# facebookresearch/CPC_audio

Hardware: AMD Instinct MI355X
Metric: audio-seconds/sec (train step) (higher is better)
Workload: dtype f32 (conv GEMMs and the GRU forward recurrence: fp32 operands as 2 scaled fp16 pieces -- the inputs of conv1/conv2 stored that way --, 3 fp16 MFMAs per product; GRU backward recurrence and the criterion's dz gather-GEMM: f32 MFMAs; InfoNCE scores: 2 fp16 pieces; other GEMMs: 3 bf16 pieces, 6 bf16 MF

## Files before the change

cpc_audio_amd/_lib.py:

```python
import ctypes
import os
import threading

_HERE = os.path.dirname(os.path.abspath(__file__))
LIB_PATH = os.path.join(_HERE, "lib", "libcpc_hip.so")
DEFAULT_GRU_MODE = 2
DEFAULT_GRU_XCD_LOCAL = 1
DEFAULT_GRU_POLL_PLAIN = 15
DEFAULT_MFMA_MODE = 3
EXPECTED_ABI = 16
DEFAULT_DMA_PIPELINE = 2
DEFAULT_WGRAD_DMA_STAGES = 4
DEFAULT_CONV_SMALL_PIPE = 1
DEFAULT_GRU_WGRAD_STREAM = 1
DEFAULT_NCE_FUSED = 2
DEFAULT_INDEX_PREP_GROUPS = -1
DEFAULT_FWD_NSPLIT = 0
DEFAULT_DGRAD_NSPLIT = 256
DEFAULT_STEP_SCHEDULE = (1, 0)

_P = ctypes.c_void_p
_I = ctypes.c_int
_L = ctypes.c_long
_F = ctypes.c_float

SIGNATURES = {
    "cpc_abi_version": (_I, []),
    "cpc_release_stream": (_I, [_P]),
    "cpc_streams_overlap": (_I, [_P, _P, _P]),
    "cpc_set_mfma_mode": (_I, [_I]),
    "cpc_get_mfma_mode": (_I, []),
    "cpc_device_error_flags": (_I, [_I]),
    "cpc_conv0_forward": (_I, [_P] * 8 + [_I, _I, _P]),
    "cpc_conv0_forward_h2": (_I, [_P] * 9 + [_I, _I, _P]),
    "cpc_h2_encode": (_I, [_P, _P, _L, _P, _P]),
    "cpc_h2_decode": (_I, [_P, _P, _L, _P, _P]),
    "cpc_conv_weight_relayout_h2": (_I, [_P, _P, _I, _P]),
    "cpc_conv_gemm_forward_h2": (_I, [_P] * 11 + [_I] * 6 + [_P]),
    "cpc_set_dma_tile": (_I, [_I]),
    "cpc_set_conv0_tuning": (_I, [_I, _I]),
    "cpc_set_h2_layers": (_I, [_I]),
    "cpc_set_h2_dx": (_I, [_I]),
    "cpc_set_wgrad1_early": (_I, [_I]),
    "cpc_set_dma_layer2": (_I, [_I]),
    "cpc_set_conv_small_tile": (_I, [_I]),
    "cpc_set_dgrad_nsplit": (_I, [_I]),
    "cpc_set_conv_small_pipe": (_I, [_I]),
    "cpc_set_wgrad_dma_groups": (_I, [_I]),
    "cpc_set_wgrad_dma_stages": (_I, [_I]),
    "cpc_set_wgrad_dma_min_rows": (_I, [_I]),
    "cpc_set_gemm_split": (_I, [_I]),
    "cpc_set_gemm_dma": (_I, [_I]),
# ... 82 lines not shown
    "cpc_pred_conv_backward": (_I, [_P] * 8 + [_I] * 5 + [_F, _I, _P]),
    "cpc_probe_layout": (_I, [_I, _I, _P]),
    "cpc_probe_train_step": (_I, [_P, _L, _P, _I, _I] + [_P] * 6 + [ctypes.c_double] * 6 + [_P] * 7),
    "cpc_probe_eval": (_I, [_P, _L, _P, _I, _I] + [_P] * 7),
    "cpc_posterior_forward": (_I, [_P, _L, _P, _P, _I, _I, _I, _P, _P, _P]),
    "cpc_abx_layout": (_I, [_I, _I, _I, _L, _P]),
    "cpc_abx_group_scores": (_I, [_P, _P, _P, _I, _L, _I, _I, _I, _P, _P, _P, _I, _P, _I, _I, _P, _P, _P]),
    "cpc_abx_pair_dtw": (_I, [_P, _P, _P, _I, _L, _I, _I, _I, _P, _I, _P, _P]),
    "cpc_abx_dtw": (_I, [_P, _P, _P, _I, _I, _I, _I, _I, _I, _P, _P]),
    "cpc_ctc_decode_layout": (_I, [_I, _I, _I, _I, _P]),
    "cpc_ctc_beam_search": (_I, [_P, _I, _L, _L, _L, _P, _I, _I, _I, _I, _I, _I, _P, _L, _P, _P, _P, _P, _P]),
    "cpc_nw_align_score": (_I, [_P, _L, _P, _I, _P, _L, _P, _I, _I, ctypes.c_double, ctypes.c_double, ctypes.c_double, _I, _P,
                                _P]),
    "cpc_nce_layout": (_I, [_I, _I, _I, _I, _P]),
    "cpc_nce_prepare": (_I, [_P] * 6 + [_I, _I, _I, _I, _P]),
    "cpc_nce_forward": (_I, [_P] * 8 + [_I, _I, _I, _I, _P]),
    "cpc_nce_forward_prepared": (_I, [_P] * 8 + [_I, _I, _I, _I, _P]),
    "cpc_nce_bounds": (_I, [_P, ctypes.c_float, _P, _P, _I, _I, _I, _I, _P]),
    "cpc_nce_forward_streams": (_I, [_P] * 8 + [_I, _I, _I, _I, _I, _P, _P]),
    "cpc_nce_backward_prepare": (_I, [_P] * 5 + [_I, _I, _I, _I, _P]),
    "cpc_nce_backward_prepared": (_I, [_P] * 10 + [_I, _I, _I, _I, _P]),
    "cpc_nce_backward": (_I, [_P] * 12 + [_I, _I, _I, _I, _P]),
    "cpc_nce_backward_streams": (_I, [_P] * 12 + [_I, _I, _I, _I, _P, _P]),
    "cpc_nce_backward_dz": (_I, [_P] * 7 + [_I, _I, _I, _I, _P]),
    "cpc_nce_backward_dwall": (_I, [_P] * 4 + [_I, _I, _I, _I, _P]),
    "cpc_set_nce_fused": (_I, [_I]),
    "cpc_get_nce_fused": (_I, []),
    "cpc_set_nce_grid": (_I, [_I]),
    "cpc_set_nce_debug": (_I, [_I]),
    "cpc_set_nce_rows_apart": (_I, [_I]),
    "cpc_set_nce_heads_dma": (_I, [_I]),
    "cpc_nce_prepare_z": (_I, [_P, _P, _I, _I, _I, _I, _P]),
    "cpc_set_index_prep_groups": (_I, [_I]),
    "cpc_set_gru_wgrad_stream": (_I, [_I]),
    "cpc_nce_padded_negatives": (_I, [_I]),
    "cpc_nce_head_group": (_I, [_I, _I]),
    "cpc_set_step_schedule": (_I, [_I, _I]),
    "cpc_train_step_layout": (_I, [_I, _I, _I, _I, _P]),
    "cpc_train_step_prefetch": (_I, [_P, _P, _P, _I, _I, _I, _I, _P]),
    "cpc_train_step": (_I, [_P, _P, _P, _P, _F] + [_P] * 7 + [_I] * 5 + [_P] * 4),
    "cpc_train_step_tail": (_I, [_P, _P, _I, _I, _I, _I, _I, _P, _P, _P]),
    "cpc_train_step_wait": (_I, [_P, _I, _P]),
    "cpc_set_fwd_nsplit": (_I, [_I, _I]),
    "cpc_set_step_timing": (_I, [_I]),
    "cpc_set_tail_schedule": (_I, [_I]),
    "cpc_get_step_timing": (_I, [_P]),
    "cpc_adam_step": (_I, [_P] * 5 + [_I] + [ctypes.c_double] * 6 + [_P]),
    "cpc_adam_step_capturable": (_I, [_P] * 5 + [_I] + [ctypes.c_double] * 4 + [_P, _P, _P]),
}


class CpcHipError(RuntimeError):
    pass


class Bound:

    def __init__(self, cdll, path):
        self.path = path
        self._cdll = cdll
        missing = []
        for name, (res, args) in SIGNATURES.items():
            try:
                fn = getattr(cdll, name)
            except AttributeError:
                missing.append(name)
# ... 56 lines not shown
```

cpc_audio_amd/csrc/cpc_internal.h:

```cpp
#pragma once
#include "cpc_common.h"
#include "gemm_tile.h"

namespace cpc {

constexpr int kRowsSumGroups = 128;
int rows_sum(const float* part, int nrows, int n, float* tmp, float* out, hipStream_t stream, int G = 1, long part_gs = 0,
             long tmp_gs = 0, long out_gs = 0);
constexpr int kRowsSumMaxJobs = 8;
struct RowsSumJob { const float* part; int nrows; int n; float* tmp; float* out; };
int rows_sum_multi(const RowsSumJob* jobs, int njobs, hipStream_t stream);

struct GemmBounds {
    const float* a = nullptr;
    const float* b = nullptr;
    int a_slots = 1, b_slots = 1;
    long a_gs = 0, b_gs = 0;
};
int absmax_slots(const float* const* x, const long* n, int njobs, float* out, hipStream_t st, const float* cval = nullptr);
int absmax_group(const float* const* x, const long* n, const long* x_gs, int njobs, int G, float* out, long out_gs, hipStream_t st);

struct GemmGroup {
    int G = 1;
    long a = 0, b = 0, bias = 0, c = 0;
// ... 92 lines not shown
                        int* splits_out, hipStream_t st);
int conv_wgrad_dma(const void* dx_h2, const void* x_h2, float* part, const float* dx_bound, const float* x_bound,
                   const float* zeros, int B, int Lin, int k, int s, int p, int* splits_out, hipStream_t st);
int bf16_decode(const void* src, float* dst, long n, hipStream_t st);
int conv0_forward_bf16(const float* wave, const float* w, const float* bias, const float* nw, const float* nb, void* y,
                       float* mean, float* rstd, int B, int L, hipStream_t st);
int conv0_backward(const float* wave, const float* w, const float* bias, const float* nw, const float* nb,
                   const float* mean, const float* rstd, const void* dy, int dy_bf16, float* scratch, float* dW0, float* dB0,
                   float* dNW0, float* dNB0, int B, int L, hipStream_t stream);

int head_row_lse(const float* logits, float* lse, int R, int C, hipStream_t st);
int head_colsum(const float* dl, float* dbp, int R, int C, int kchunk, int Z, hipStream_t st);
constexpr int kCtcNone = 0, kCtcMean = 1, kCtcSum = 2;
int ctc_loss_saved_floats(int B, int T, int C, int Lmax, long* floats);
int ctc_loss_forward(const float* logits, const long long* in_len, const long long* targets, long tgt_stride,
                     const long long* tgt_len, float* saved, float* loss, int B, int T, int C, int Lmax, int blank, int reduction,
                     hipStream_t st);
int ctc_loss_backward(const float* logits, const float* saved, const float* dloss, float* dlogits, int B, int T, int C, int Lmax,
                      int blank, int reduction, hipStream_t st);

template <class T>
int device_flag_fetch(T& sym, int clear, unsigned* out) {
    unsigned v = 0;
    if (hipMemcpyFromSymbol(&v, sym, sizeof(v)) != hipSuccess) return CPC_ERR_ARG;
    if (clear && v) {
        const unsigned zero = 0;
        if (hipMemcpyToSymbol(sym, &zero, sizeof(zero)) != hipSuccess) return CPC_ERR_ARG;
    }
    *out = v;
    return 0;
}
int gru_error_flag_fetch(int clear, unsigned* out);
int nce_error_flag_fetch(int clear, unsigned* out);
int enc_error_flag_fetch(int clear, unsigned* out);
int lstm_error_flag_fetch(int clear, unsigned* out);
int sup_error_flag_fetch(int clear, unsigned* out);
int probe_error_flag_fetch(int clear, unsigned* out);
int abx_error_flag_fetch(int clear, unsigned* out);
int decode_error_flag_fetch(int clear, unsigned* out);
int ctc_error_flag_fetch(int clear, unsigned* out);
int seqnorm_error_flag_fetch(int clear, unsigned* out);
int rnn_error_flag_fetch(int clear, unsigned* out);

static inline long align64l(long v) { return (v + 63) & ~63L; }

}
```

cpc_audio_amd/csrc/nce.hip:

```cpp
#include <algorithm>
#include "cpc_common.h"
#include "cpc_internal.h"
#include "gemm_tile.h"

namespace cpc {

__device__ __forceinline__ float4 ld4(const float* p) { return *reinterpret_cast<const float4*>(p); }
__device__ __forceinline__ float dot4(const float4& a, const float4& b) {
    return fmaf(a.x, b.x, fmaf(a.y, b.y, fmaf(a.z, b.z, a.w * b.w)));
}

struct Gather16 {
    float4 v[4][4];
    __device__ __forceinline__ void issue(const float* const (&rowp)[4]) {
#pragma unroll
        for (int q = 0; q < 4; ++q)
#pragma unroll
            for (int g = 0; g < 4; ++g) v[q][g] = ld4(rowp[q] + 64 * g);
    }
    __device__ __forceinline__ void block(int g, float4* tile, float4 (&out)[4]) const {
        const int lane = threadIdx.x & 63, c = lane & 15, r4 = lane >> 4;
        __builtin_amdgcn_wave_barrier();
#pragma unroll
        for (int q = 0; q < 4; ++q) tile[(4 * q + r4) * 16 + (c ^ (4 * q + r4))] = v[q][g];
// ... 1110 lines not shown
__global__ __launch_bounds__(1024) void nce_scan_kernel(const int* __restrict__ count, int* __restrict__ row_ptr,
                                                        int* __restrict__ cursor, int n) {
    __shared__ int part[1024];
    const int tid = threadIdx.x;
    const int per = (n + 1023) / 1024;
    const int lo = tid * per, hi = min(n, lo + per);
    int s = 0;
    for (int i = lo; i < hi; ++i) s += count[i];
    part[tid] = s;
    __syncthreads();
    for (int off = 1; off < 1024; off <<= 1) {
        const int v = tid >= off ? part[tid - off] : 0;
        __syncthreads();
        part[tid] += v;
        __syncthreads();
    }
    int run = part[tid] - s;
    for (int i = lo; i < hi; ++i) {
        row_ptr[i] = run;
        cursor[i] = run;
        run += count[i];
    }
    if (tid == 1023) row_ptr[n] = part[1023];
}

__global__ __launch_bounds__(256) void nce_fill_kernel(const int* __restrict__ dest, int* __restrict__ cursor,
                                                       int* __restrict__ perm, long total) {
    for (long slot = (long)blockIdx.x * 256 + threadIdx.x; slot < total; slot += (long)gridDim.x * 256) {
        const int pos = atomicAdd(&cursor[dest[slot]], 1);
        perm[pos] = (int)slot;
    }
}

int g_index_prep_groups = -1;
int g_nce_fused = 2;
int g_nce_heads_dma = 1;
int g_nce_dbg = 0;
int g_nce_rows_apart = 1;
int g_nce_grid = -1;

struct NceLayout {
    int W, BW;
    int koff;
    int N, Nv;
    long pred, logits, lse, bounds, tpred, ps, zh, chf, wqh, saved_total;
    long rowstat, tmp, sums, fwd_total;
    long dpred, wallT, part, gscale, V, dS, G, wcat, part_dz, ch, bwd_total;
};

constexpr int kDzSplits = 4;

static thread_local int g_head_off = 0, g_head_total = 0;
static thread_local bool g_zh_ready = false;
static thread_local bool g_wqh_ready = false;

static bool nce_layout(int B, int S, int K, int N, NceLayout& n) {
    const int Ktot = g_head_total > 0 ? g_head_total : K;
    if (B <= 0 || K <= 0 || K > 16 || g_head_off + K > Ktot || S <= Ktot || N <= 0) return false;
    n.Nv = N;
    N = (N + 15) & ~15;
    n.N = N;
    n.koff = g_head_total > 0 ? g_head_off : 0;
    n.W = S - Ktot;
    n.BW = B * n.W;
    long o = 0;
    n.pred = o; o += align64l((long)n.BW * K * kC);
// ... 145 lines not shown
    if (h2) { gb.a = bnd + 128; gb.a_slots = kAmaxSlots; gb.b = bnd + 18; }
    SplitK sk;
    sk.part = scratch + n.part_dz;
    sk.floats = (long)kDzSplits * B * S * kC;
    return nt_gemm(plain_rows(G, B * S, K * kC), wcat, K * kC, nullptr, dz, kC, kC, K * kC, st, 0, 0, gb, GemmGroup(), sk);
}

__global__ __launch_bounds__(256) void nce_scale_tpred_kernel(const float* __restrict__ T, const float* __restrict__ gscale,
                                                              float* __restrict__ dpred, long n4, int K) {
    const long i = (long)blockIdx.x * 256 + threadIdx.x;
    if (i >= n4) return;
    const float g = gscale[(int)((i / (kC / 4)) % K)];
    float4 v = reinterpret_cast<const float4*>(T)[i];
    v.x *= g; v.y *= g; v.z *= g; v.w *= g;
    reinterpret_cast<float4*>(dpred)[i] = v;
}

static int nce_scores_backward(const NceLayout& n, const float* z, const int* ext, const float* saved, const float* gloss,
                               float* scratch, float* dpred, int B, int S, int K, int N, hipStream_t st,
                               const float* fwd_bounds = nullptr, float* dc_tail = nullptr, float* dS = nullptr,
                               bool gscale_done = false) {
    const float* logits = saved + n.logits, *lse = saved + n.lse;
    float* gscale = scratch + n.gscale;
    const float gs = 1.0f / ((float)n.BW * (float)kC);
    if (!gscale_done)
    hipLaunchKernelGGL(nce_gscale_kernel, dim3(dc_tail ? 1 + 128 : 1), dim3(64), 0, st, gloss, gscale, K, gs, fwd_bounds, dc_tail, B,
                       S, n.W);
    hipLaunchKernelGGL(nce_bwd_dpred_kernel, dim3(cdiv(n.BW, 4)), dim3(256), 0, st, z, ext, logits, lse, gscale, dpred, n.BW,
                       n.W, S, K, N, fwd_bounds ? gscale + 64 : (float*)nullptr, dS, n.koff);
    CPC_LAUNCH_CHECK();
    return 0;
}

int nce_error_flag_fetch(int clear, unsigned* out) { return device_flag_fetch(HIP_SYMBOL(g_nce_bad_index), clear, out); }

}

using namespace cpc;

extern "C" int cpc_nce_layout(int B, int S, int K, int N, long* sizes) {
    NceLayout n;
    CPC_RETURN_IF(!nce_layout(B, S, K, N, n), CPC_ERR_SHAPE);
    N = n.N;
    sizes[0] = n.saved_total; sizes[1] = n.fwd_total; sizes[2] = n.bwd_total;
    sizes[3] = n.pred; sizes[4] = n.logits; sizes[5] = n.lse;
    return 0;
}

extern "C" int cpc_nce_padded_negatives(int N) { return N <= 0 ? 0 : (N + 15) & ~15; }

extern "C" int cpc_nce_prepare(const long* batchIdx, const long* seqIdx, int* ext, int* perm, int* row_ptr,
                               int* work, int B, int S, int K, int N, void* stream) {
    NceLayout n;
    CPC_RETURN_IF(!nce_layout(B, S, K, N, n), CPC_ERR_SHAPE);
    N = n.N;
    CPC_RETURN_IF(!batchIdx || !seqIdx || !ext || !perm || !row_ptr || !work, CPC_ERR_ARG);
    hipStream_t st = (hipStream_t)stream;
    const long total = (long)n.BW * (N + K);
    const int rows = B * S;
    int* dest = work;
    int* count = work + total;
    int* cursor = count + rows + 1;
    (void)hipMemsetAsync(count, 0, sizeof(int) * (rows + 1), st);
    long cap = g_index_prep_groups;
    if (cap < 0) {
        int dev = 0, cus = 0;
        if (hipGetDevice(&dev) != hipSuccess || hipDeviceGetAttribute(&cus, hipDeviceAttributeMultiprocessorCount, dev) != hipSuccess) cus = 0;
        cap = cus;
    }
    const auto capped = [cap](long wgs) { return (unsigned)(cap > 0 ? std::min<long>(wgs, cap) : wgs); };
    hipLaunchKernelGGL(nce_rows_kernel, dim3(capped(cdiv(n.BW, 4))), dim3(256), 0, st, batchIdx, seqIdx, ext, B, S, n.W, n.Nv, N);
    hipLaunchKernelGGL(nce_index_kernel, dim3(capped(cdiv(total, 256))), dim3(256), 0, st, ext, dest, count, B, S, n.W, K, N, n.koff);
    hipLaunchKernelGGL(nce_scan_kernel, dim3(1), dim3(1024), 0, st, count, row_ptr, cursor, rows);
    hipLaunchKernelGGL(nce_fill_kernel, dim3(capped(cdiv(total, 256))), dim3(256), 0, st, dest, cursor, perm, total);
    CPC_LAUNCH_CHECK();
    return 0;
}

static int nce_forward(const float* c, const float* z, const float* wall, const int* ext, float* saved, float* scratch,
                       float* losses, float* acc, int B, int S, int K, int N, hipStream_t st, bool bounds_ready,
                       hipStream_t fin = nullptr) {
    NceLayout n;
    CPC_RETURN_IF(!nce_layout(B, S, K, N, n), CPC_ERR_SHAPE);
    N = n.N;
    CPC_RETURN_IF(!c || !z || !wall || !ext || !saved || !scratch || !losses || !acc, CPC_ERR_ARG);
    float* pred = saved + n.pred;
    if (!bounds_ready) {
        const float* xs[3] = {c, wall, nullptr};
        const long ns[3] = {(long)B * S * kC, (long)K * kC * kC, 0};
        int rc = absmax_slots(xs, ns, 3, saved + n.bounds, st);
        if (rc) return rc;
    }
    GemmBounds gb;
    gb.a = saved + n.bounds; gb.a_slots = kAmaxSlots;
    gb.b = saved + n.bounds + kAmaxSlots; gb.b_slots = kAmaxSlots;
    int rc = 0;
    if (nce_heads_dma(K)) {
        if (!(bounds_ready && g_wqh_ready))
            rc = gemm_weight_h2(wall, kC, 1, K * kC, kC, saved + n.wqh, saved + n.bounds + kAmaxSlots, nullptr, 1, 0, 0, 0, 0, st);
        g_wqh_ready = false;
        if (rc) return rc;
        rc = nce_rows_to_h2(c, saved + n.chf, saved + n.bounds, (long)B * S, st);
// ... 191 lines not shown
}

extern "C" int cpc_nce_backward_dwall(const float* c, const float* saved, float* scratch, float* dwall, int B, int S, int K,
                                      int N, void* stream) {
    NceLayout n;
    CPC_RETURN_IF(!nce_layout(B, S, K, N, n), CPC_ERR_SHAPE);
    N = n.N;
    CPC_RETURN_IF(!c || !saved || !scratch || !dwall, CPC_ERR_ARG);
    const bool fused = nce_fused(N) != 0;
    GemmBounds gdw;
    GemmGroup grp;
    if (g_mfma_mode >= 2) {
        gdw.a = fused ? saved + n.bounds + 2 * kAmaxSlots : scratch + n.gscale + 64; gdw.a_slots = kAmaxSlots;
        gdw.b = scratch + n.gscale + 17;
    }
    if (fused) { grp.out_scale = scratch + n.gscale; grp.out_scale_rows = kC; }
    return tn_gemm(plain_rows(fused ? saved + n.tpred : scratch + n.dpred, n.BW, K * kC), K * kC, window_rows(c, B, S, n.W), kC,
                   scratch + n.part, dwall, 0, (hipStream_t)stream, gdw, grp);
}

extern "C" int cpc_nce_head_group(int k0, int k_total) {
    CPC_RETURN_IF(k0 < 0 || k_total < 0 || (k_total == 0 && k0 != 0) || (k_total > 0 && k0 >= k_total), CPC_ERR_ARG);
    g_head_off = k0;
    g_head_total = k_total;
    return 0;
}

extern "C" int cpc_set_index_prep_groups(int n) {
    CPC_RETURN_IF(n < -1, CPC_ERR_ARG);
    g_index_prep_groups = n;
    return 0;
}

extern "C" int cpc_set_nce_fused(int on) {
    CPC_RETURN_IF(on < 0 || on > 3, CPC_ERR_ARG);
    g_nce_fused = on;
    return 0;
}
extern "C" int cpc_get_nce_fused(void) { return g_nce_fused; }
extern "C" int cpc_set_nce_heads_dma(int on) { g_nce_heads_dma = on ? 1 : 0; return 0; }
extern "C" int cpc_set_nce_rows_apart(int on) { g_nce_rows_apart = on ? 1 : 0; return 0; }
extern "C" int cpc_set_nce_debug(int mask) { g_nce_dbg = mask; return 0; }

extern "C" int cpc_set_nce_grid(int wgs) {
    CPC_RETURN_IF(wgs < -1, CPC_ERR_ARG);
    g_nce_grid = wgs;
    return 0;
}

extern "C" int cpc_nce_prepare_z(const float* z, float* saved, int B, int S, int K, int N, void* stream) {
    NceLayout n;
    CPC_RETURN_IF(!nce_layout(B, S, K, N, n), CPC_ERR_SHAPE);
    CPC_RETURN_IF(!z || !saved, CPC_ERR_ARG);
    if (nce_fused(n.N) < 2) return 0;
    g_zh_ready = true;
    return nce_prepare_zh(n, z, saved, B, S, (hipStream_t)stream);
}
```

cpc_audio_amd/csrc/train_step.hip:

```cpp
#include "cpc_common.h"
#include "cpc_internal.h"

namespace cpc {
namespace {

constexpr int kEncParams = 20, kGruParams = 8;

struct StepLayout {
    int S, W;
    long enc[22], gru[3], nce[6], coef;
    long enc_saved, enc_fscr, z, gru_saved, gru_fscr, c, gcoef, nce_saved, nce_fscr, ext, perm, row_ptr, work;
    long nce_bscr, dc, dz, gru_bscr, dx, enc_bscr, total;
};

bool step_layout(int B, int L, int K, int N, StepLayout& s) {
    if (B <= 0 || cpc_encoder_layout(B, L, s.enc) != 0) return false;
    s.S = (int)s.enc[7];
    s.W = s.S - K;
    if (s.W <= 0 || cpc_gru_layout(B, s.S, 2, s.gru) != 0 || cpc_nce_layout(B, s.S, K, N, s.nce) != 0) return false;
    s.coef = cpc_gru_coef_floats(B, s.S, 2);
    if (s.coef <= 0) return false;
    const int Np = cpc_nce_padded_negatives(N);
    const long act = (long)B * s.S * kC, slots = (long)B * s.W * (Np + K), rows = (long)B * s.S;
    long o = 0;
    auto take = [&](long n) { const long at = o; o += align64l(n); return at; };
    s.enc_saved = take(s.enc[0]); s.enc_fscr = take(std::max(1L, s.enc[1])); s.z = take(act);
    s.gru_saved = take(s.gru[0]); s.gru_fscr = take(s.gru[1]); s.c = take(act); s.gcoef = take(s.coef);
    s.nce_saved = take(s.nce[0]); s.nce_fscr = take(s.nce[1]);
    s.ext = take((long)B * s.W * Np); s.perm = take(slots); s.row_ptr = take(rows + 1); s.work = take(slots + 2 * rows + 2);
    s.nce_bscr = take(s.nce[2]); s.dc = take(act); s.dz = take(act);
    s.gru_bscr = take(s.gru[2]); s.dx = take(act); s.enc_bscr = take(s.enc[2]);
    s.total = o;
    return true;
}

__global__ __launch_bounds__(256) void add_inplace_kernel(float* __restrict__ a, const float* __restrict__ b, long n4) {
    const long i = (long)blockIdx.x * 256 + threadIdx.x;
    if (i >= n4) return;
    float4 x = reinterpret_cast<float4*>(a)[i];
    const float4 y = reinterpret_cast<const float4*>(b)[i];
    x.x += y.x; x.y += y.y; x.z += y.z; x.w += y.w;
    reinterpret_cast<float4*>(a)[i] = x;
}

int g_prep_point = 1;
int g_no_early = 0;
int g_weight_prep_apart = 0;
int g_gru_wgrad_prep = 1;
int g_dz_early = 0;

inline bool rec(hipEvent_t e, hipStream_t s) { return hipEventRecord(e, s) == hipSuccess; }
inline bool wait(hipStream_t s, hipEvent_t e) { return hipStreamWaitEvent(s, e, 0) == hipSuccess; }

int g_step_timing = 0;
hipEvent_t g_timers[10];
bool g_timers_made = false;

struct HookScope {
    StepHooks saved;
    HookScope() : saved(step_hooks()) {}
    ~HookScope() { step_hooks() = saved; }
};

}

void enc_set_after_conv0_event(hipEvent_t ev);
void enc_set_forward_event(int layer, hipEvent_t ev);
void enc_set_weight_prep_stream(hipStream_t st, hipEvent_t done);

}

using namespace cpc;

extern "C" int cpc_set_gru_wgrad_stream(int on_prep) {
    g_gru_wgrad_prep = on_prep ? 1 : 0;
    return 0;
}

extern "C" int cpc_set_step_schedule(int prep_point, int dz_early) {
    CPC_RETURN_IF(prep_point < 0 || prep_point > 3 || dz_early < 0 || dz_early > 7, CPC_ERR_ARG);
    g_prep_point = prep_point;
    g_dz_early = dz_early & 1;
    g_no_early = (dz_early >> 1) & 1;
    g_weight_prep_apart = (dz_early >> 2) & 1;
    return 0;
}

extern "C" int cpc_train_step_layout(int B, int L, int K, int N, long* sizes) {
    StepLayout s;
    CPC_RETURN_IF(!sizes || !step_layout(B, L, K, N, s), CPC_ERR_SHAPE);
    sizes[0] = s.total; sizes[1] = s.z; sizes[2] = s.c; sizes[3] = s.S;
    sizes[4] = s.ext; sizes[5] = s.dz; sizes[6] = s.dc; sizes[7] = s.dx;
    return 0;
}

extern "C" int cpc_train_step(const float* wave, const long* batchIdx, const long* seqIdx, const float* h0, float c_bound,
                              const float* const* params, float* const* grads, const float* gloss, float* workspace,
                              float* losses, float* acc, float* hN, int B, int L, int K, int N, int phases, void* main_stream,
                              void* side_stream, void* prep_stream, void* wgrad_stream) {
    StepLayout s;
    CPC_RETURN_IF(!step_layout(B, L, K, N, s), CPC_ERR_SHAPE);
    CPC_RETURN_IF(!wave || !params || !grads || !workspace || (phases & ~31) || !(phases & 3), CPC_ERR_ARG);
    CPC_RETURN_IF(((phases & 4) && !(phases & 2)) || ((phases & 8) && !(phases & 1)), CPC_ERR_ARG);
    hipStream_t M = (hipStream_t)main_stream, S0 = (hipStream_t)side_stream, S1 = (hipStream_t)prep_stream,
                S2 = (hipStream_t)wgrad_stream;
    hipEvent_t* pool = stream_events(M);
    CPC_RETURN_IF(!pool, CPC_ERR_ARG);
    HookScope scope;
    StepHooks& hk = step_hooks();
    hk.parity = (phases & 16) ? 1 : 0;
    hk.weights_ready = (phases & 8) != 0;
    hk.conv1_wait[0] = (phases & 8) ? pool[kEvNextConv1] : nullptr;
    hk.conv1_wait[1] = (phases & 8) ? pool[kEvNextRest] : nullptr;
    hk.open_tail = (phases & 4) != 0 && S2 != M;
    hk.sums_stream = hk.open_tail && S1 != M ? S1 : nullptr;
    hk.timers = (g_step_timing && g_timers_made) ? g_timers : nullptr;
    hipEvent_t* ev = pool + 12;
    float* ws = workspace;
    const float* const* enc_p = params;
    const float* const* gru_p = params + kEncParams;
    const float* wall = params[kEncParams + kGruParams];
    float* const* enc_g = grads;
    float* const* gru_g = grads + kEncParams;
    float* dwall = grads[kEncParams + kGruParams];
    float* z = ws + s.z, *c = ws + s.c, *coef = ws + s.gcoef, *dz = ws + s.dz, *dc = ws + s.dc, *dx = ws + s.dx;
    int* ext = reinterpret_cast<int*>(ws + s.ext), *perm = reinterpret_cast<int*>(ws + s.perm);
    int* row_ptr = reinterpret_cast<int*>(ws + s.row_ptr), *work = reinterpret_cast<int*>(ws + s.work);
    const int S = s.S;
    int rc = 0;
    if (phases & 1) {
        CPC_RETURN_IF((batchIdx == nullptr) != (seqIdx == nullptr) || !gloss || !losses || !acc || !hN, CPC_ERR_ARG);
        CPC_RETURN_IF(!rec(ev[0], M) || !wait(S1, ev[0]), CPC_ERR_ARG);
        if (phases & 8) CPC_RETURN_IF(!wait(S0, pool[kEvNextRest]), CPC_ERR_ARG);
        const bool bounds_early = c_bound > 0.f;
        const bool early = bounds_early && !g_no_early;
        auto prepare = [&]() -> int {
            int r = batchIdx ? cpc_nce_prepare(batchIdx, seqIdx, ext, perm, row_ptr, work, B, S, K, N, S0) : 0;
            if (r) return r;
            if (bounds_early) r = cpc_nce_bounds(nullptr, c_bound, wall, ws + s.nce_saved, B, S, K, N, S0);
            if (r) return r;
            if (early) r = cpc_nce_backward_prepare(wall, ws + s.nce_saved, gloss, ws + s.nce_bscr, dc, B, S, K, N, S0);
            if (r) return r;
            return rec(ev[1], S0) ? 0 : CPC_ERR_ARG;
        };
        if (g_prep_point == 0) {
            CPC_RETURN_IF(!wait(S0, ev[0]), CPC_ERR_ARG);
            if ((rc = prepare())) return rc;
        }
        if (g_prep_point == 3) enc_set_forward_event(1, ev[6]);
        else enc_set_after_conv0_event(g_prep_point == 1 ? ev[6] : nullptr);
        enc_set_weight_prep_stream(g_weight_prep_apart ? S1 : nullptr, ev[8]);
        rc = cpc_encoder_forward(wave, enc_p, ws + s.enc_saved, ws + s.enc_fscr, z, B, L, M);
        enc_set_after_conv0_event(nullptr);
        enc_set_weight_prep_stream(nullptr, nullptr);
        if (rc) return rc;
        rc = cpc_gru_forward_prepare(ws + s.gru_fscr, B, S, 2, S1);
        if (rc) return rc;
        CPC_RETURN_IF(!rec(ev[7], S1), CPC_ERR_ARG);
        if (g_prep_point == 1 || g_prep_point == 3) {
            CPC_RETURN_IF(!wait(S0, ev[6]), CPC_ERR_ARG);
            if ((rc = prepare())) return rc;
        } else if (g_prep_point == 2) {
            CPC_RETURN_IF(!rec(ev[6], M) || !wait(S0, ev[6]), CPC_ERR_ARG);
            if ((rc = prepare())) return rc;
        }
        if (cpc_get_nce_fused() >= 2 && S0 != M) {
            CPC_RETURN_IF(!rec(pool[kEvEncoderDone], M) || !wait(S0, pool[kEvEncoderDone]), CPC_ERR_ARG);
            rc = cpc_nce_prepare_z(z, ws + s.nce_saved, B, S, K, N, S0);
            if (rc) return rc;
            CPC_RETURN_IF(!rec(ev[1], S0), CPC_ERR_ARG);
        }
        CPC_RETURN_IF(!wait(M, ev[7]), CPC_ERR_ARG);
        rc = cpc_gru_forward_coef_prepared(z, h0, gru_p, ws + s.gru_saved, ws + s.gru_fscr, c, hN, coef, B, S, 2, M);
        if (rc) return rc;
        rc = cpc_gru_backward_coef(h0, gru_p, ws + s.gru_saved, c, coef, 1, B, S, 2, S1);
        if (rc) return rc;
        CPC_RETURN_IF(!rec(ev[2], S1) || !wait(M, ev[1]), CPC_ERR_ARG);
        rc = cpc_nce_forward_streams(c, z, wall, ext, ws + s.nce_saved, ws + s.nce_fscr, losses, acc, B, S, K, N, bounds_early ? 1 : 0, M,
                                     early && !g_dz_early ? S0 : M);
        if (rc) return rc;
        rc = early ? cpc_nce_backward_prepared(c, z, wall, ext, perm, row_ptr, ws + s.nce_saved, gloss, ws + s.nce_bscr, dc, B, S, K,
                                               N, M)
                   : cpc_nce_backward_streams(c, z, wall, ext, perm, row_ptr, ws + s.nce_saved, gloss, ws + s.nce_bscr, dc, nullptr,
                                              nullptr, B, S, K, N, M, M);
        if (rc) return rc;
        if (g_dz_early) {
            rc = cpc_nce_backward_dz(c, wall, perm, row_ptr, ws + s.nce_saved, ws + s.nce_bscr, dz, B, S, K, N, M);
            if (rc) return rc;
        }
        step_timer_mark(5, M);
        CPC_RETURN_IF(!rec(ev[3], M) || !wait(M, ev[2]), CPC_ERR_ARG);
        const bool gru_wgrad_prep = g_gru_wgrad_prep && (phases & 3) == 3 && S1 != M && S1 != S2;
        rc = cpc_gru_backward_streams(z, h0, gru_p, ws + s.gru_saved, c, dc, coef, ws + s.gru_bscr, dx, gru_g, B, S, 2, M,
                                      gru_wgrad_prep ? S1 : S2);
        if (rc) return rc;
// ... 94 lines not shown
```

include/cpc_hip.h:

```cpp
#ifndef CPC_HIP_H
#define CPC_HIP_H

#ifdef __cplusplus
extern "C" {
#endif

#define CPC_OK 0
#define CPC_ERR_SHAPE 1
#define CPC_ERR_ARG 2

int cpc_abi_version(void);
int cpc_release_stream(void* stream);
int cpc_streams_overlap(void* stream_a, void* stream_b, int* overlap);

int cpc_set_mfma_mode(int mode);
int cpc_get_mfma_mode(void);

#define CPC_DEVERR_GRU_POLL_TIMEOUT 1
#define CPC_DEVERR_NEGATIVE_INDEX 2
#define CPC_DEVERR_CONV_EXCHANGE 4
#define CPC_DEVERR_LSTM_POLL_TIMEOUT 8
#define CPC_DEVERR_LABEL_RANGE 16
#define CPC_DEVERR_ABX_INDEX 32
#define CPC_DEVERR_DECODE_RANGE 64
// ... 236 lines not shown
int cpc_nce_forward_prepared(const float* c, const float* z, const float* wall, const int* ext, float* saved,
                             float* scratch, float* losses, float* acc, int B, int S, int K, int N, void* stream);
int cpc_nce_forward_streams(const float* c, const float* z, const float* wall, const int* ext, float* saved, float* scratch,
                            float* losses, float* acc, int B, int S, int K, int N, int bounds_ready, void* stream,
                            void* finalize_stream);
int cpc_nce_backward_prepare(const float* wall, const float* saved, const float* gloss, float* scratch, float* dc, int B, int S,
                             int K, int N, void* stream);
int cpc_nce_backward_prepared(const float* c, const float* z, const float* wall, const int* ext, const int* perm,
                              const int* row_ptr, const float* saved, const float* gloss, float* scratch, float* dc, int B,
                              int S, int K, int N, void* stream);
int cpc_nce_backward(const float* c, const float* z, const float* wall, const int* ext,
                     const int* perm, const int* row_ptr, const float* saved, const float* gloss,
                     float* scratch, float* dc, float* dz, float* dwall, int B, int S, int K, int N,
                     void* stream);

int cpc_nce_backward_streams(const float* c, const float* z, const float* wall, const int* ext,
                             const int* perm, const int* row_ptr, const float* saved, const float* gloss,
                             float* scratch, float* dc, float* dz, float* dwall, int B, int S, int K, int N,
                             void* stream, void* dz_stream);

int cpc_nce_backward_dz(const float* c, const float* wall, const int* perm, const int* row_ptr, const float* saved,
                        float* scratch, float* dz, int B, int S, int K, int N, void* stream);

int cpc_nce_backward_dwall(const float* c, const float* saved, float* scratch, float* dwall, int B, int S, int K, int N,
                           void* stream);
int cpc_set_nce_fused(int on);
int cpc_get_nce_fused(void);
int cpc_set_nce_grid(int wgs);
int cpc_set_nce_rows_apart(int on);
int cpc_set_nce_heads_dma(int on);
int cpc_set_nce_debug(int mask);
int cpc_nce_prepare_z(const float* z, float* saved, int B, int S, int K, int N, void* stream);
int cpc_set_index_prep_groups(int n);
int cpc_set_gru_wgrad_stream(int on_prep);

int cpc_nce_scores_forward(const float* pred, const float* z, const int* ext, float* saved, float* scratch,
                           float* losses, float* acc, int B, int S, int K, int N, void* stream);
int cpc_nce_scores_backward(const float* pred, const float* z, const int* ext, const int* perm,
                            const int* row_ptr, const float* saved, const float* gloss, float* scratch,
                            float* dpred, float* dz, int B, int S, int K, int N, void* stream);

int cpc_train_step_layout(int B, int L, int K, int N, long* sizes);
int cpc_train_step(const float* wave, const long* batchIdx, const long* seqIdx, const float* h0, float c_bound,
                   const float* const* params, float* const* grads, const float* gloss, float* workspace, float* losses,
                   float* acc, float* hN, int B, int L, int K, int N, int phases, void* main_stream, void* side_stream,
                   void* prep_stream, void* wgrad_stream);
int cpc_train_step_prefetch(const long* batchIdx, const long* seqIdx, float* workspace, int B, int L, int K, int N,
                            void* side_stream);
int cpc_train_step_tail(const float* const* params, float* workspace, int B, int L, int K, int N, int next_parity,
                        void* main_stream, void* prep_stream, void* wgrad_stream);
int cpc_train_step_wait(void* main_stream, int which, void* waiting_stream);
int cpc_set_fwd_nsplit(int min_wgs, int spin_limit);
int cpc_set_step_timing(int on);
int cpc_set_tail_schedule(int conv0_early);
int cpc_get_step_timing(float* us);
int cpc_set_step_schedule(int prep_point, int dz_early);

int cpc_adam_step(float* const* params, const float* const* grads, float* const* exp_avg, float* const* exp_avg_sq,
                  const long* numel, int n, double lr, double beta1, double beta2, double eps, double bias_correction1,
                  double bias_correction2_sqrt, void* stream);
int cpc_adam_step_capturable(float* const* params, const float* const* grads, float* const* exp_avg,
                             float* const* exp_avg_sq, const long* numel, int n, double lr, double beta1, double beta2,
                             double eps, double* step, float* coef, void* stream);

#ifdef __cplusplus
}
// ... 3 lines not shown
```

Before: 31490.

## Build NCE negative-index CSR with per-group LDS histograms and move prep point

Replaces the global-atomic counting-sort index preparation (memset, rows, index, scan, fill kernels) with a three-kernel scheme. Each workgroup builds its own LDS histogram (packed 16-bit when rows exceed the wide limit) and bitonic-sorts each window's negatives in LDS. Per-group offsets come from a two-level scan, and the fill kernel scatters with LDS atomics, aiming to cut global atomic contention and launch count. The step schedule now defaults to an auto prep point that launches index prep after the encoder forward when the LDS path applies, which changes the overlap with other streams.

```diff
diff --git a/cpc_audio_amd/_lib.py b/cpc_audio_amd/_lib.py
--- a/cpc_audio_amd/_lib.py
+++ b/cpc_audio_amd/_lib.py
@@ -15,9 +15,10 @@
 DEFAULT_GRU_WGRAD_STREAM = 1
 DEFAULT_NCE_FUSED = 2
 DEFAULT_INDEX_PREP_GROUPS = -1
+DEFAULT_INDEX_PREP_MODE = 1
 DEFAULT_FWD_NSPLIT = 0
 DEFAULT_DGRAD_NSPLIT = 256
-DEFAULT_STEP_SCHEDULE = (1, 0)
+DEFAULT_STEP_SCHEDULE = (-1, 0)
 
 _P = ctypes.c_void_p
 _I = ctypes.c_int
@@ -166,6 +167,7 @@
     "cpc_set_nce_heads_dma": (_I, [_I]),
     "cpc_nce_prepare_z": (_I, [_P, _P, _I, _I, _I, _I, _P]),
     "cpc_set_index_prep_groups": (_I, [_I]),
+    "cpc_set_index_prep_mode": (_I, [_I]),
     "cpc_set_gru_wgrad_stream": (_I, [_I]),
     "cpc_nce_padded_negatives": (_I, [_I]),
     "cpc_nce_head_group": (_I, [_I, _I]),
diff --git a/cpc_audio_amd/csrc/cpc_internal.h b/cpc_audio_amd/csrc/cpc_internal.h
--- a/cpc_audio_amd/csrc/cpc_internal.h
+++ b/cpc_audio_amd/csrc/cpc_internal.h
@@ -148,6 +148,7 @@
 }
 int gru_error_flag_fetch(int clear, unsigned* out);
 int nce_error_flag_fetch(int clear, unsigned* out);
+bool nce_index_prep_in_lds(int B, int S, int K, int N);
 int enc_error_flag_fetch(int clear, unsigned* out);
 int lstm_error_flag_fetch(int clear, unsigned* out);
 int sup_error_flag_fetch(int clear, unsigned* out);
diff --git a/cpc_audio_amd/csrc/nce.hip b/cpc_audio_amd/csrc/nce.hip
--- a/cpc_audio_amd/csrc/nce.hip
+++ b/cpc_audio_amd/csrc/nce.hip
@@ -1166,6 +1166,205 @@
     }
 }
 
+constexpr int kPrepThreads = 1024;
+constexpr int kPrepTile = 8192;
+constexpr int kPrepHistWords = 8192;
+constexpr int kPrepOffRows = 128;
+constexpr int kPrepOffSegs = 8;
+
+template <bool Wide>
+static __device__ __forceinline__ int prep_count(unsigned* h, int d) {
+    if (Wide) return (int)atomicAdd(&h[d], 1u);
+    const int sh = (d & 1) * 16;
+    return (int)((atomicAdd(&h[d >> 1], 1u << sh) >> sh) & 0xffffu);
+}
+template <bool Wide>
+static __device__ __forceinline__ int prep_counted(const unsigned* h, int d) {
+    return Wide ? (int)h[d] : (int)((h[d >> 1] >> ((d & 1) * 16)) & 0xffffu);
+}
+
+template <bool Wide>
+__global__ __launch_bounds__(kPrepThreads) void nce_prep_rows_kernel(const long* __restrict__ batchIdx, const long* __restrict__ seqIdx,
+                                                                     int* __restrict__ ext, int* __restrict__ hist,
+                                                                     int* __restrict__ bsum, int B, int S, int W, int N, int Np, int K,
+                                                                     int koff, int per) {
+    __shared__ int tile[kPrepTile + 128];
+    __shared__ unsigned h[kPrepHistWords];
+    constexpr int kWaves = kPrepThreads / 64;
+    const int tid = threadIdx.x, lane = tid & 63, wv = tid >> 6;
+    const int rows = B * S, BW = B * W, G = gridDim.x, g = blockIdx.x;
+    const int w0 = min(BW, g * per), w1 = min(BW, w0 + per);
+    for (int i = tid; i < (Wide ? rows : (rows + 1) / 2); i += kPrepThreads) h[i] = 0u;
+    const bool sort = N <= kSortMax;
+    int P = 64;
+    while (P < N && P < kSortMax) P <<= 1;
+    int lgT = 0;
+    while ((P << (lgT + 1)) <= kPrepTile) ++lgT;
+    if (!sort || lgT > 6) lgT = 6;
+    const int T = 1 << lgT, pitch = P + 1;
+    const int extra = Np - N + K;
+    __syncthreads();
+    for (int c0 = w0; c0 < w1; c0 += T) {
+        const int nw = min(T, w1 - c0);
+        for (int i = tid; i < (N << lgT); i += kPrepThreads) {
+            const int e = i & (T - 1), j = i >> lgT;
+            if (e >= nw) continue;
+            const int bt = c0 + e, b = bt / W, t = bt - b * W;
+            const long flat = ((long)b * N + j) * W + t;
+            long si = seqIdx[flat], bi = batchIdx[flat];
+            if (si < 0 || si >= S || bi < 0 || bi >= B) {
+                atomicOr(&g_nce_bad_index, 1u);
+                si = si < 0 ? 0 : (si >= S ? S - 1 : si);
+                bi = bi < 0 ? 0 : (bi >= B ? B - 1 : bi);
+            }
+            int r = (int)si + t;
+            if (r >= S) r -= S;
+            const int d = r + (int)bi * S;
+            if (sort) {
+                tile[e * pitch + j] = d;
+            } else {
+                ext[(long)bt * Np + j] = d;
+                prep_count<Wide>(h, d);
+            }
+        }
+        for (int i = tid; i < nw * extra; i += kPrepThreads) {
+            const int e = i / extra, j = i - e * extra;
+            const int bt = c0 + e, b = bt / W, t = bt - b * W;
+            int d = b * S + t;
+            if (j < Np - N) ext[(long)bt * Np + N + j] = d;
+            else d += koff + (j - (Np - N)) + 1;
+            prep_count<Wide>(h, d);
+        }
+        if (!sort) continue;
+        __syncthreads();
+        for (int e = wv; e < nw; e += kWaves)
+            for (int j = N + lane; j < P; j += 64) tile[e * pitch + j] = 0x7fffffff;
+        __builtin_amdgcn_wave_barrier();
+        for (int k = 2; k <= P; k <<= 1) {
+            for (int j = k >> 1; j > 0; j >>= 1) {
+                for (int pr = lane; pr < P / 2; pr += 64) {
+                    const int i = ((pr & ~(j - 1)) << 1) | (pr & (j - 1)), q = i + j;
+                    const bool up = (i & k) == 0;
+                    for (int e0 = wv; e0 < nw; e0 += 4 * kWaves) {
+                        int a[4], c[4];
+#pragma unroll
+                        for (int u = 0; u < 4; ++u) {
+                            const int e = e0 + u * kWaves;
+                            if (e < nw) { a[u] = tile[e * pitch + i]; c[u] = tile[e * pitch + q]; }
+                        }
+#pragma unroll
+                        for (int u = 0; u < 4; ++u) {
+                            const int e = e0 + u * kWaves;
+                            if (e < nw && (a[u] > c[u]) == up) { tile[e * pitch + i] = c[u]; tile[e * pitch + q] = a[u]; }
+                        }
+                    }
+                }
+                __builtin_amdgcn_wave_barrier();
+            }
+        }
+        for (int e = wv; e < nw; e += kWaves) {
+            const int* __restrict__ r = tile + e * pitch;
+            int* __restrict__ out = ext + (long)(c0 + e) * Np;
+            for (int j = lane; j < N; j += 64) {
+                const int d = r[j];
+                out[j] = d;
+                prep_count<Wide>(h, d);
+            }
+        }
+        __syncthreads();
+    }
+    __syncthreads();
+    for (int d = tid; d < rows; d += kPrepThreads) hist[(long)g * rows + d] = prep_counted<Wide>(h, d);
+    const int R = (rows + kPrepOffRows - 1) / kPrepOffRows;
+    for (int r = wv; r < R; r += kWaves) {
+        int s = 0;
+        for (int d = r * kPrepOffRows + lane; d < min(rows, (r + 1) * kPrepOffRows); d += 64) s += prep_counted<Wide>(h, d);
+        for (int m = 32; m > 0; m >>= 1) s += __shfl_xor(s, m);
+        if (lane == 0) bsum[r * G + g] = s;
+    }
+}
+
+__global__ __launch_bounds__(kPrepOffRows * kPrepOffSegs) void nce_prep_offsets_kernel(int* __restrict__ hist, const int* __restrict__ bsum,
+                                                                                       int* __restrict__ row_ptr, int rows, int G) {
+    constexpr int kThreads = kPrepOffRows * kPrepOffSegs, kWaves = kThreads / 64, kRowWaves = kPrepOffRows / 64;
+    __shared__ int segsum[kPrepOffSegs][kPrepOffRows];
+    __shared__ int wbase[kWaves], wtot[kWaves];
+    const int tid = threadIdx.x, lane = tid & 63, wv = tid >> 6;
+    const int row = tid % kPrepOffRows, seg = tid / kPrepOffRows;
+    const int r = blockIdx.x, d = r * kPrepOffRows + row;
+    const int gper = (G + kPrepOffSegs - 1) / kPrepOffSegs, g0 = min(G, seg * gper), g1 = min(G, g0 + gper);
+    int s = 0;
+    for (int i = tid; i < r * G; i += kThreads) s += bsum[i];
+    for (int m = 32; m > 0; m >>= 1) s += __shfl_xor(s, m);
+    if (lane == 0) wbase[wv] = s;
+    int part = 0;
+    if (d < rows)
+        for (int g = g0; g < g1; ++g) part += hist[(long)g * rows + d];
+    segsum[seg][row] = part;
+    __syncthreads();
+    int tot = 0, before = 0;
+    for (int q = 0; q < kPrepOffSegs; ++q) {
+        const int v = segsum[q][row];
+        tot += v;
+        if (q < seg) before += v;
+    }
+    int inc = tot;
+    for (int off = 1; off < 64; off <<= 1) {
+        const int v = __shfl_up(inc, off);
+        if (lane >= off) inc += v;
+    }
+    if (lane == 63) wtot[wv] = inc;
+    __syncthreads();
+    int start = inc - tot;
+    for (int w = 0; w < kWaves; ++w) start += wbase[w];
+    for (int w = wv - wv % kRowWaves; w < wv; ++w) start += wtot[w];
+    if (d >= rows) return;
+    if (seg == 0) {
+        row_ptr[d] = start;
+        if (d == rows - 1) row_ptr[rows] = start + tot;
+    }
+    int run = start + before;
+    for (int g = g0; g < g1; g += 8) {
+        int v[8];
+#pragma unroll
+        for (int u = 0; u < 8; ++u) v[u] = g + u < g1 ? hist[(long)(g + u) * rows + d] : 0;
+#pragma unroll
+        for (int u = 0; u < 8; ++u)
+            if (g + u < g1) {
+                hist[(long)(g + u) * rows + d] = run;
+                run += v[u];
+            }
+    }
+}
+
+template <bool Wide>
+__global__ __launch_bounds__(kPrepThreads) void nce_prep_fill_kernel(const int* __restrict__ ext, const int* __restrict__ hist,
+                                                                     int* __restrict__ perm, int B, int S, int W, int Np, int K,
+                                                                     int koff, int per) {
+    __shared__ unsigned cur[kPrepHistWords];
+    const int tid = threadIdx.x;
+    const int rows = B * S, BW = B * W, g = blockIdx.x;
+    const int w0 = min(BW, g * per), w1 = min(BW, w0 + per);
+    const int* __restrict__ first = hist + (long)g * rows;
+    if (Wide) for (int i = tid; i < rows; i += kPrepThreads) cur[i] = (unsigned)first[i];
+    else for (int i = tid; i < (rows + 1) / 2; i += kPrepThreads) cur[i] = 0u;
+    __syncthreads();
+    const int C = Np + K;
+    for (long slot = (long)w0 * C + tid; slot < (long)w1 * C; slot += kPrepThreads) {
+        const int bt = (int)(slot / C), j = (int)(slot - (long)bt * C);
+        int d;
+        if (j < Np) {
+            d = ext[(long)bt * Np + j];
+        } else {
+            const int b = bt / W, t = bt - b * W;
+            d = b * S + t + koff + (j - Np) + 1;
+        }
+        const int pos = Wide ? prep_count<true>(cur, d) : first[d] + prep_count<false>(cur, d);
+        perm[pos] = (int)slot;
+    }
+}
+
+int g_index_prep_mode = 1;
 int g_index_prep_groups = -1;
 int g_nce_fused = 2;
 int g_nce_heads_dma = 1;
@@ -1377,6 +1576,36 @@
     return 0;
 }
 
+static long prep_group_cap() {
+    long cap = g_index_prep_groups;
+    if (cap < 0) {
+        int dev = 0, cus = 0;
+        if (hipGetDevice(&dev) != hipSuccess || hipDeviceGetAttribute(&cus, hipDeviceAttributeMultiprocessorCount, dev) != hipSuccess) cus = 0;
+        cap = cus;
+    }
+    return cap;
+}
+
+struct PrepPlan { int G, per; bool wide; };
+static bool prep_plan(const NceLayout& n, int B, int K, long cap, PrepPlan& pl) {
+    const long rows = (long)B * (n.W + (g_head_total > 0 ? g_head_total : K)), total = (long)n.BW * (n.N + K);
+    if (g_index_prep_mode != 1 || rows > 2 * kPrepHistWords) return false;
+    const long R = cdiv(rows, kPrepOffRows);
+    long G = std::min<long>(std::min<long>(total / rows, (2 * rows + 2) / R), n.BW);
+    if (cap > 0) G = std::min(G, cap);
+    if (G < 1) return false;
+    pl.per = cdiv(n.BW, G);
+    pl.G = cdiv(n.BW, pl.per);
+    pl.wide = rows <= kPrepHistWords;
+    return pl.wide || (long)pl.per * (n.N + K) < 65536;
+}
+
+bool nce_index_prep_in_lds(int B, int S, int K, int N) {
+    NceLayout n;
+    PrepPlan pl;
+    return nce_layout(B, S, K, N, n) && prep_plan(n, B, K, prep_group_cap(), pl);
+}
+
 int nce_error_flag_fetch(int clear, unsigned* out) { return device_flag_fetch(HIP_SYMBOL(g_nce_bad_index), clear, out); }
 
 }
@@ -1403,16 +1632,30 @@
     hipStream_t st = (hipStream_t)stream;
     const long total = (long)n.BW * (N + K);
     const int rows = B * S;
+    const long cap = prep_group_cap();
+    PrepPlan pl;
+    if (prep_plan(n, B, K, cap, pl)) {
+        int* hist = work;
+        int* bsum = work + total;
+        const dim3 grid((unsigned)pl.G), offs((unsigned)cdiv(rows, kPrepOffRows));
+        if (pl.wide) {
+            hipLaunchKernelGGL(nce_prep_rows_kernel<true>, grid, dim3(kPrepThreads), 0, st, batchIdx, seqIdx, ext, hist, bsum, B, S, n.W, n.Nv,
+                               N, K, n.koff, pl.per);
+            hipLaunchKernelGGL(nce_prep_offsets_kernel, offs, dim3(kPrepOffRows * kPrepOffSegs), 0, st, hist, bsum, row_ptr, rows, pl.G);
+            hipLaunchKernelGGL(nce_prep_fill_kernel<true>, grid, dim3(kPrepThreads), 0, st, ext, hist, perm, B, S, n.W, N, K, n.koff, pl.per);
+        } else {
+            hipLaunchKernelGGL(nce_prep_rows_kernel<false>, grid, dim3(kPrepThreads), 0, st, batchIdx, seqIdx, ext, hist, bsum, B, S, n.W, n.Nv,
+                               N, K, n.koff, pl.per);
+            hipLaunchKernelGGL(nce_prep_offsets_kernel, offs, dim3(kPrepOffRows * kPrepOffSegs), 0, st, hist, bsum, row_ptr, rows, pl.G);
+            hipLaunchKernelGGL(nce_prep_fill_kernel<false>, grid, dim3(kPrepThreads), 0, st, ext, hist, perm, B, S, n.W, N, K, n.koff, pl.per);
+        }
+        CPC_LAUNCH_CHECK();
+        return 0;
+    }
     int* dest = work;
     int* count = work + total;
     int* cursor = count + rows + 1;
     (void)hipMemsetAsync(count, 0, sizeof(int) * (rows + 1), st);
-    long cap = g_index_prep_groups;
-    if (cap < 0) {
-        int dev = 0, cus = 0;
-        if (hipGetDevice(&dev) != hipSuccess || hipDeviceGetAttribute(&cus, hipDeviceAttributeMultiprocessorCount, dev) != hipSuccess) cus = 0;
-        cap = cus;
-    }
     const auto capped = [cap](long wgs) { return (unsigned)(cap > 0 ? std::min<long>(wgs, cap) : wgs); };
     hipLaunchKernelGGL(nce_rows_kernel, dim3(capped(cdiv(n.BW, 4))), dim3(256), 0, st, batchIdx, seqIdx, ext, B, S, n.W, n.Nv, N);
     hipLaunchKernelGGL(nce_index_kernel, dim3(capped(cdiv(total, 256))), dim3(256), 0, st, ext, dest, count, B, S, n.W, K, N, n.koff);
@@ -1670,6 +1913,12 @@
     return 0;
 }
 
+extern "C" int cpc_set_index_prep_mode(int mode) {
+    CPC_RETURN_IF(mode < 0 || mode > 1, CPC_ERR_ARG);
+    g_index_prep_mode = mode;
+    return 0;
+}
+
 extern "C" int cpc_set_nce_fused(int on) {
     CPC_RETURN_IF(on < 0 || on > 3, CPC_ERR_ARG);
     g_nce_fused = on;
diff --git a/cpc_audio_amd/csrc/train_step.hip b/cpc_audio_amd/csrc/train_step.hip
--- a/cpc_audio_amd/csrc/train_step.hip
+++ b/cpc_audio_amd/csrc/train_step.hip
@@ -43,7 +43,7 @@
     reinterpret_cast<float4*>(a)[i] = x;
 }
 
-int g_prep_point = 1;
+int g_prep_point = -1;
 int g_no_early = 0;
 int g_weight_prep_apart = 0;
 int g_gru_wgrad_prep = 1;
@@ -78,7 +78,7 @@
 }
 
 extern "C" int cpc_set_step_schedule(int prep_point, int dz_early) {
-    CPC_RETURN_IF(prep_point < 0 || prep_point > 3 || dz_early < 0 || dz_early > 7, CPC_ERR_ARG);
+    CPC_RETURN_IF(prep_point < -1 || prep_point > 3 || dz_early < 0 || dz_early > 7, CPC_ERR_ARG);
     g_prep_point = prep_point;
     g_dz_early = dz_early & 1;
     g_no_early = (dz_early >> 1) & 1;
@@ -143,12 +143,13 @@
             if (r) return r;
             return rec(ev[1], S0) ? 0 : CPC_ERR_ARG;
         };
-        if (g_prep_point == 0) {
+        const int point = g_prep_point >= 0 ? g_prep_point : (nce_index_prep_in_lds(B, S, K, N) ? 3 : 1);
+        if (point == 0) {
             CPC_RETURN_IF(!wait(S0, ev[0]), CPC_ERR_ARG);
             if ((rc = prepare())) return rc;
         }
-        if (g_prep_point == 3) enc_set_forward_event(1, ev[6]);
-        else enc_set_after_conv0_event(g_prep_point == 1 ? ev[6] : nullptr);
+        if (point == 3) enc_set_forward_event(1, ev[6]);
+        else enc_set_after_conv0_event(point == 1 ? ev[6] : nullptr);
         enc_set_weight_prep_stream(g_weight_prep_apart ? S1 : nullptr, ev[8]);
         rc = cpc_encoder_forward(wave, enc_p, ws + s.enc_saved, ws + s.enc_fscr, z, B, L, M);
         enc_set_after_conv0_event(nullptr);
@@ -157,10 +158,10 @@
         rc = cpc_gru_forward_prepare(ws + s.gru_fscr, B, S, 2, S1);
         if (rc) return rc;
         CPC_RETURN_IF(!rec(ev[7], S1), CPC_ERR_ARG);
-        if (g_prep_point == 1 || g_prep_point == 3) {
+        if (point == 1 || point == 3) {
             CPC_RETURN_IF(!wait(S0, ev[6]), CPC_ERR_ARG);
             if ((rc = prepare())) return rc;
-        } else if (g_prep_point == 2) {
+        } else if (point == 2) {
             CPC_RETURN_IF(!rec(ev[6], M) || !wait(S0, ev[6]), CPC_ERR_ARG);
             if ((rc = prepare())) return rc;
         }
diff --git a/include/cpc_hip.h b/include/cpc_hip.h
--- a/include/cpc_hip.h
+++ b/include/cpc_hip.h
@@ -292,6 +292,7 @@
 int cpc_set_nce_debug(int mask);
 int cpc_nce_prepare_z(const float* z, float* saved, int B, int S, int K, int N, void* stream);
 int cpc_set_index_prep_groups(int n);
+int cpc_set_index_prep_mode(int mode);
 int cpc_set_gru_wgrad_stream(int on_prep);
 
 int cpc_nce_scores_forward(const float* pred, const float* z, const int* ext, float* saved, float* scratch,
```

After: 31780 (median of 6 runs). Within noise of the previous version (+0.9%).
